# rogerhh/MonoGS

Hardware: AMD Instinct MI355X
Metric: rasteriser fwd+bwd fps @640x480/300k Gaussians (higher is better)
Workload: dtype f32; 1 GPU; SYN-C: 300000 Gaussians @ 640x480, SH degree 0, fwd+bwd incl. pose Jacobian through the autograd binding; pairs_D=750233, autograd_multithreading=False, parallelism=single view

## Files before the change

monogs_amd/csrc/raster_forward.hip:

```cpp
#include <type_traits>

#include "launch.h"
#include "raster_kernels.h"
#include "objective_math.h"
#define MGS_DIAG_FORWARD
#include "diag_stamp.h"

namespace mgs {

__device__ __forceinline__ void load_camera(Camera& c, const KP& P) {
#pragma unroll
  for (int i = 0; i < 16; i++) { c.V[i] = P.V[i]; c.PM[i] = P.PM[i]; c.Praw[i] = P.Praw[i]; }
  c.campos[0] = P.campos[0]; c.campos[1] = P.campos[1]; c.campos[2] = P.campos[2];
  c.W = P.W; c.H = P.H; c.tanfovx = P.tanfovx; c.tanfovy = P.tanfovy;
  c.focal_x = P.focal_x; c.focal_y = P.focal_y; c.scale_modifier = P.mod;
  c.sh_degree = P.deg; c.sh_coeffs = P.K; c.grid_x = P.grid_x; c.grid_y = P.grid_y;
  c.clamp_grad_upstream = P.clamp_up;
}

__device__ __forceinline__ void project_and_store(const KP& P, int idx, float4& r0, float4& r1) {
  Camera cam;
  load_camera(cam, P);
  const float p[3] = {P.means[3 * idx], P.means[3 * idx + 1], P.means[3 * idx + 2]};
  const float* pcol = P.precol ? P.precol + (size_t)3 * idx : nullptr;
// ... 186 lines not shown
          const int pos = P.tile_offset[t] + atomicAdd(&P.tile_cursor[t], 1);
          if (pos < P.cap) {
            P.keys[pos] = keyhi | (unsigned int)idx;
            P.payload[pos] = (unsigned int)cnt;
          }
        } else {
          atomicAdd(&P.tile_count[t], 1);
        }
        cnt++;
      }
    }
  }
  if (!emit) P.pair_count[idx] = cnt;
}

__global__ __launch_bounds__(256) void k_scan_reduce(KP P) {
  __shared__ int s[256];
  const int tid = threadIdx.x;
  const int base = blockIdx.x * kScanBlock + tid * 8;
  int sum = 0;
#pragma unroll
  for (int i = 0; i < 8; i++) sum += (base + i < P.N) ? P.pair_count[base + i] : 0;
  s[tid] = sum;
  __syncthreads();
  for (int off = 128; off > 0; off >>= 1) {
    if (tid < off) s[tid] += s[tid + off];
    __syncthreads();
  }
  if (tid == 0) P.scan_tmp[blockIdx.x] = s[0];
}

__global__ __launch_bounds__(1024) void k_scan_sums(KP P, int nblk) {
  __shared__ int s[1024];
  const int tid = threadIdx.x;
  int carry = 0;
  for (int base = 0; base < nblk; base += 1024) {
    const int i = base + tid;
    const int v = (i < nblk) ? P.scan_tmp[i] : 0;
    s[tid] = v;
    __syncthreads();
    for (int off = 1; off < 1024; off <<= 1) {
      const int t = (tid >= off) ? s[tid - off] : 0;
      __syncthreads();
      s[tid] += t;
      __syncthreads();
    }
    if (i < nblk) P.scan_tmp[i] = carry + s[tid] - v;
    carry += s[1023];
    __syncthreads();
  }
  if (tid == 0) P.scan_tmp[nblk] = carry;
}

__global__ __launch_bounds__(256) void k_scan_write(KP P) {
  __shared__ int s[256];
  const int tid = threadIdx.x;
  const int base = blockIdx.x * kScanBlock + tid * 8;
  int v[8], sum = 0;
#pragma unroll
  for (int i = 0; i < 8; i++) { v[i] = (base + i < P.N) ? P.pair_count[base + i] : 0; sum += v[i]; }
  s[tid] = sum;
  __syncthreads();
  for (int off = 1; off < 256; off <<= 1) {
    const int t = (tid >= off) ? s[tid - off] : 0;
    __syncthreads();
    s[tid] += t;
    __syncthreads();
  }
  int run = P.scan_tmp[blockIdx.x] + s[tid] - sum;
#pragma unroll
  for (int i = 0; i < 8; i++) {
    if (base + i < P.N) P.pair_off[base + i] = run;
    run += v[i];
  }
}

__device__ __forceinline__ void tile_scan_body(const KP& P, int nbin, int* s_sum, int* s_seg) {
  int* s_w = s_sum;
  const int tid = threadIdx.x, lane = tid & 63, wave = tid >> 6;
  const int vb = (nbin > 0 && tid < nbin) ? P.scan_tmp[tid] : 0;
  const int per = (P.T + 1023) / 1024;
  const int lo = tid * per, hi = min(lo + per, P.T);
  int local = 0, lseg = 0, lmax = 0;
  for (int i = lo; i < hi; i++) {
    const int c = __hip_atomic_load(&P.tile_count[i], __ATOMIC_RELAXED, __HIP_MEMORY_SCOPE_AGENT);
    local += c;
    lseg += (c + kItem - 1) / kItem;
    lmax = max(lmax, c);
  }
  int ib = vb, ip = local, is = lseg;
#pragma unroll
  for (int off = 1; off < 64; off <<= 1) {
    const int tb = __shfl_up(ib, off), tp = __shfl_up(ip, off), ts = __shfl_up(is, off);
    if (lane >= off) { ib += tb; ip += tp; is += ts; }
  }
#pragma unroll
  for (int off = 32; off > 0; off >>= 1) lmax = max(lmax, __shfl_xor(lmax, off));
  __syncthreads();
  if (lane == 63) { s_w[wave] = ib; s_w[16 + wave] = ip; s_w[32 + wave] = is; s_w[48 + wave] = lmax; }
  __syncthreads();
  int ob = 0, op = 0, os = 0, tot_p = 0, tot_s = 0, tmax = 0;
#pragma unroll
  for (int w = 0; w < 16; w++) {
    const int xb = s_w[w], xp = s_w[16 + w], xs = s_w[32 + w];
    if (w < wave) { ob += xb; op += xp; os += xs; }
    tot_p += xp; tot_s += xs;
    tmax = max(tmax, s_w[48 + w]);
  }
  if (nbin > 0) {
    if (tid < nbin) P.block_prefix[tid] = ob + ib - vb;
  } else if (tid == 0) {
    P.block_prefix[0] = 0;
  }
  int run = op + ip - local, rseg = os + is - lseg;
  for (int i = lo; i < hi; i++) {
    const int c = __hip_atomic_load(&P.tile_count[i], __ATOMIC_RELAXED, __HIP_MEMORY_SCOPE_AGENT);
    P.tile_offset[i] = run;
    P.seg_offset[i] = rseg;
    run += c;
    rseg += (c + kItem - 1) / kItem;
  }
  if (tid == 1023) {
    P.tile_offset[P.T] = tot_p;
    P.seg_offset[P.T] = tot_s;
    P.counters[0] = tot_p;
    if (P.d_out) {
      __hip_atomic_store(P.d_out + 1, tmax, __ATOMIC_RELAXED, __HIP_MEMORY_SCOPE_SYSTEM);
      __hip_atomic_store(P.d_out, tot_p, __ATOMIC_RELAXED, __HIP_MEMORY_SCOPE_SYSTEM);
    }
    P.counters[1] = tot_s;
    if (P.d_max) atomicMax(P.d_max, tot_p);
  }
  (void)s_seg;
}

__global__ __launch_bounds__(1024) void k_tile_scan(KP P, int nbin) {
  __shared__ int s_sum[1024], s_seg[1024];
  tile_scan_body(P, nbin, s_sum, s_seg);
}

constexpr int kColGroups = 16;
constexpr int kColRows = kBinBlocks / kColGroups;

__global__ __launch_bounds__(64 * kColGroups) void k_bin_colsum(KP P, int nblk) {
  __shared__ int s_sum2[2048];
  int (*s_sum)[64] = reinterpret_cast<int (*)[64]>(s_sum2);
  const int tl = threadIdx.x & 63, grp = threadIdx.x >> 6;
  const int t = blockIdx.x * 64 + tl;
  int v[kColRows];
  int sum = 0;
#pragma unroll
  for (int i = 0; i < kColRows; i++) {
    const int b = grp * kColRows + i;
    v[i] = (t < P.T && b < nblk) ? P.bin_table[(size_t)b * P.T + t] : 0;
    sum += v[i];
  }
  s_sum[grp][tl] = sum;
  __syncthreads();
  int run = 0, tot = 0;
#pragma unroll
  for (int g = 0; g < kColGroups; g++) {
    const int x = s_sum[g][tl];
    if (g < grp) run += x;
    tot += x;
  }
  if (t < P.T) {
#pragma unroll
    for (int i = 0; i < kColRows; i++) {
      const int b = grp * kColRows + i;
      if (b < nblk) P.bin_table[(size_t)b * P.T + t] = run;
      run += v[i];
    }
    if (grp == 0) __hip_atomic_store(&P.tile_count[t], tot, __ATOMIC_RELAXED, __HIP_MEMORY_SCOPE_AGENT);
  }
  __shared__ int s_last;
  if (threadIdx.x < 64) {
    asm volatile("s_waitcnt vmcnt(0)" ::: "memory");
    if (threadIdx.x == 0) {
      const int ticket = atomicAdd(&P.counters[3], 1);
      s_last = ticket == (int)gridDim.x - 1;
    }
  }
  __syncthreads();
  if (!s_last) return;
  tile_scan_body(P, nblk, s_sum2, s_sum2 + 1024);
}


template <bool WAVE_LOCAL, bool HAS_VAL, int NWAVES, typename KP_, typename VP_>
__device__ __forceinline__ void bitonic_sort(KP_ key, VP_ val, int n, int tid) {
  int m = 2;
  while (m < n) m <<= 1;
  const int half_m = m >> 1;
  const int nw = WAVE_LOCAL ? max(1, min(NWAVES, m >> 7)) : NWAVES;
  const int chunk = m / nw;
  const int cpw = half_m / nw;
  const int wave = tid >> 6, lane = tid & 63;
  const bool active = wave < nw;
  bool prev_global = true;
  auto sync = [&](bool global) {
    if (!WAVE_LOCAL || global || prev_global) {
      __syncthreads();
    } else {
      __builtin_amdgcn_fence(__ATOMIC_ACQ_REL, "wavefront");
      __builtin_amdgcn_wave_barrier();
    }
    prev_global = global;
  };
  constexpr int kMaxCmp = 2;
  auto run = [&](auto&& pair_of) {
    for (int c0 = 0; c0 < cpw; c0 += 64 * kMaxCmp) {
      int lo[kMaxCmp], hi[kMaxCmp];
      unsigned long long a[kMaxCmp], b[kMaxCmp];
      unsigned int va[kMaxCmp], vb[kMaxCmp];
#pragma unroll
      for (int u = 0; u < kMaxCmp; u++) {
        const int c = c0 + lane + 64 * u;
        lo[u] = -1;
        if (c < cpw) {
          pair_of(wave * cpw + c, lo[u], hi[u]);
          if (hi[u] >= n) lo[u] = -1;
        }
        if (lo[u] >= 0) {
          a[u] = key[lo[u]]; b[u] = key[hi[u]];
          if constexpr (HAS_VAL) { va[u] = val[lo[u]]; vb[u] = val[hi[u]]; }
        }
      }
#pragma unroll
      for (int u = 0; u < kMaxCmp; u++) {
        if (lo[u] >= 0 && a[u] > b[u]) {
          key[lo[u]] = b[u]; key[hi[u]] = a[u];
          if constexpr (HAS_VAL) { val[lo[u]] = vb[u]; val[hi[u]] = va[u]; }
        }
      }
    }
  };
  auto reg_pass = [&](bool first_rounds) {
    constexpr unsigned long long kInf = ~0ull;
    for (int e0 = 4 * lane; e0 < chunk; e0 += 256) {
      const int b0 = wave * chunk + e0;
      if (b0 >= n) continue;
      unsigned long long k4[4];
      unsigned int v4[4];
#pragma unroll
      for (int i = 0; i < 4; i++) {
        k4[i] = b0 + i < n ? key[b0 + i] : kInf;
        if constexpr (HAS_VAL) v4[i] = b0 + i < n ? val[b0 + i] : 0u;
      }
      auto ce = [&](int a, int b) {
        if (k4[a] > k4[b]) {
          const unsigned long long t = k4[a]; k4[a] = k4[b]; k4[b] = t;
          if constexpr (HAS_VAL) { const unsigned int u = v4[a]; v4[a] = v4[b]; v4[b] = u; }
        }
      };
      if (first_rounds) { ce(0, 1); ce(2, 3); ce(0, 3); ce(1, 2); ce(0, 1); ce(2, 3); }
      else { ce(0, 2); ce(1, 3); ce(0, 1); ce(2, 3); }
#pragma unroll
      for (int i = 0; i < 4; i++) {
        if (b0 + i < n) {
          key[b0 + i] = k4[i];
          if constexpr (HAS_VAL) val[b0 + i] = v4[i];
        }
      }
// ... 427 lines not shown
      for (int c = 0; c < 3; c++) {
        float dh;
        float r = om * (gain * im[c] + bias - gt[c]);
        if constexpr (DEPTH) r *= PD.w_rgb;
        l1 += fabsf(r);
        const float h = huber(r, P.obj.huber_delta, dh);
        float phi, gam;
        norm_terms(h, P.obj.p1 ? 1.f : 2.f, phi, gam);
        acc += phi;
        float gr = gam * dh * om;
        if constexpr (DEPTH) gr *= PD.w_rgb;
        ga += gr * im[c];
        gb += gr;
        P.obj.grad_image[c * HW + pix] = gr * gain;
      }
      if constexpr (DEPTH) {
        const float gtd = PD.gt_depth[pix];
        const float dm = (gtd > PD.depth_thr && 1.f - T > PD.opa_thr) ? 1.f : 0.f;
        const float rd = PD.w_depth * (C2D.y * dm - gtd * dm);
        float dh, phi, gam;
        l1 += fabsf(rd);
        const float h = huber(rd, P.obj.huber_delta, dh);
        norm_terms(h, P.obj.p1 ? 1.f : 2.f, phi, gam);
        acc += phi;
        PD.grad_depth[pix] = gam * dh * PD.w_depth * dm;
      }
    }
#pragma unroll
    for (int off = 32; off > 0; off >>= 1) {
      acc += __shfl_down(acc, off); ga += __shfl_down(ga, off); gb += __shfl_down(gb, off); l1 += __shfl_down(l1, off);
    }
    if (lane == 0) {
      const size_t n = 4 * (size_t)P.T;
      const float sgn = a > 0.f ? 1.f : (a < 0.f ? -1.f : 0.f);
      P.obj.partial[item] = acc;
      P.obj.partial[n + item] = ga * sgn;
      P.obj.partial[2 * n + item] = gb;
      P.obj.partial[3 * n + item] = l1;
    }
  }
}

template <bool OBJ>
__global__ __launch_bounds__(64, 6) void k_blend_fwd(KP P) { blend_fwd<OBJ, false>(P, KObjDepth{}); }

__global__ __launch_bounds__(64, 6) void k_blend_fwd_rgbd(KP P, KObjDepth PD) { blend_fwd<true, true>(P, PD); }

static inline int check_launch() {
  return launches_ok() ? MGS_OK : MGS_ERR_LAUNCH;
}

static inline int num_cus() {
  static int cus = 0;
  if (cus == 0) {
    int dev = 0, v = 0;
    cus = (hipGetDevice(&dev) == hipSuccess &&
           hipDeviceGetAttribute(&v, hipDeviceAttributeMultiprocessorCount, dev) == hipSuccess && v > 0) ? v : 256;
  }
  return cus;
}

static inline int bin_blocks(int N) {
  if (N <= kBinSmallMap) return max(1, (N + 255) / 256);
  int b = max(1, min(kBinBlocks, (N + 1023) / 1024));
  const int cus = num_cus();
  if (b > cus) b = b / cus * cus;
  return b;
}

void bin_grid(int N, int& nblk, int& per) {
  const int b = bin_blocks(N);
  per = ((N + b - 1) / b + kPreBlock - 1) / kPreBlock * kPreBlock;
  nblk = (N + per - 1) / per;
}

int launch_forward_project(const KP& P, hipStream_t st) {
  if (P.T <= kBinMaxTilesLds) {
    int nblk, per;
    bin_grid(P.N, nblk, per);
    if (P.N <= kBinSmallMap)
      launch_smem("project_bin_count", k_bin_lds<256>, dim3(nblk), dim3(256), sizeof(int) * (size_t)P.T, st, P, 0, per, 1);
    else
      launch_smem("project_bin_count", k_bin_lds<1024>, dim3(nblk), dim3(1024), sizeof(int) * (size_t)P.T, st, P, 0, per, 1);
    launch("bin_colsum", k_bin_colsum, dim3((P.T + 63) / 64), dim3(64 * kColGroups), st, P, nblk);
  } else {
    launch("preprocess", k_preprocess, dim3((P.N + kPreBlock - 1) / kPreBlock), dim3(kPreBlock), st, P);
    launch("bin_count", k_bin, dim3((P.N + 255) / 256), dim3(256), st, P, 0);
    const int nscan = (P.N + kScanBlock - 1) / kScanBlock;
    launch("scan_reduce", k_scan_reduce, dim3(nscan), dim3(256), st, P);
    launch("scan_sums", k_scan_sums, dim3(1), dim3(1024), st, P, nscan);
    launch("scan_write", k_scan_write, dim3(nscan), dim3(256), st, P);
    launch("tile_scan", k_tile_scan, dim3(1), dim3(1024), st, P, 0);
  }
  return check_launch();
}

int launch_forward_blend(const KP& P, hipStream_t st, const KObjDepth* PD) {
  if (P.T <= kBinMaxTilesLds) {
    int nblk, per;
    bin_grid(P.N, nblk, per);
    if (P.N <= kBinSmallMap)
      launch_smem("bin_emit", k_bin_lds<256>, dim3(nblk), dim3(256), sizeof(int) * (size_t)P.T, st, P, 1, per, 0);
    else
      launch_smem("bin_emit", k_bin_lds<1024>, dim3(nblk), dim3(1024), sizeof(int) * (size_t)P.T, st, P, 1, per, 0);
  } else {
    if (!hip_ok("memset(tile cursors)", hipMemsetAsync(P.tile_cursor, 0, sizeof(int) * (size_t)P.T, st)) ||
        !hip_ok("memset(n_touched)", hipMemsetAsync(P.n_touched, 0, sizeof(int) * (size_t)P.N, st))) {
      launches_ok();
      return MGS_ERR_LAUNCH;
    }
    launch("bin_emit", k_bin, dim3((P.N + 255) / 256), dim3(256), st, P, 1);
  }
  if (P.pack) {
    launch("tile_sort", k_tile_sort_reg<true>, dim3(P.T), dim3(256), st, P);
    if (P.big_pass) launch("tile_sort_big", k_tile_sort<4096, 1024, true, 1024>, dim3(min(P.T, 512)), dim3(1024), st, P);
  } else {
    launch("tile_sort", k_tile_sort_reg<false>, dim3(P.T), dim3(256), st, P);
    if (P.big_pass) launch("tile_sort_big", k_tile_sort<4096, 1024, false, 1024>, dim3(min(P.T, 512)), dim3(1024), st, P);
  }
#ifdef MGS_FWD_BLOCKS
  constexpr int kFwdGridChunk = 64;
#else
  constexpr int kFwdGridChunk = kFwdChunk;
#endif
  if (P.obj.on && PD && PD->gt_depth)
    launch("blend_fwd_rgbd", k_blend_fwd_rgbd, dim3(grid_pad(4 * P.T, kFwdGridChunk)), dim3(64), st, P, *PD);
  else if (P.obj.on) launch("blend_fwd", k_blend_fwd<true>, dim3(grid_pad(4 * P.T, kFwdGridChunk)), dim3(64), st, P);
  else launch("blend_fwd", k_blend_fwd<false>, dim3(grid_pad(4 * P.T, kFwdGridChunk)), dim3(64), st, P);
  return check_launch();
}

}
```

monogs_amd/csrc/tracking.hip:

```cpp
#include <hip/hip_runtime.h>

#include "../../include/monogs_raster.h"
#include "launch.h"
#include "objective_math.h"
#include "sketch_kernels.h"

namespace mgs {

__device__ inline void so3_exp_V(const float th[3], float R[9], float V[9]) {
  const float x = th[0], y = th[1], z = th[2];
  const float W[9] = {0.f, -z, y, z, 0.f, -x, -y, x, 0.f};
  float W2[9];
  for (int i = 0; i < 3; i++)
    for (int j = 0; j < 3; j++)
      W2[3 * i + j] = W[3 * i] * W[j] + W[3 * i + 1] * W[3 + j] + W[3 * i + 2] * W[6 + j];
  const float angle = sqrtf(x * x + y * y + z * z);
  float a, b, c, d;
  if (angle < 1e-5f) {
    a = 1.f; b = 0.5f; c = 0.5f; d = 1.f / 6.f;
  } else {
    const float s = sinf(angle), co = cosf(angle), a2 = angle * angle;
    a = s / angle; b = (1.f - co) / a2; c = b; d = (angle - s) / (a2 * angle);
  }
  for (int i = 0; i < 9; i++) {
// ... 124 lines not shown
#pragma unroll
    for (int i = 0; i < len[g]; i++) {
      const int o = first[g] + i;
      if (!on[o]) continue;
      m[o] = A.beta1 * m[o] + (1.f - A.beta1) * gr[o];
      v[o] = A.beta2 * v[o] + (1.f - A.beta2) * gr[o] * gr[o];
      const float denom = sqrtf(v[o]) / bc2s + A.eps;
      p[o] -= (lr[g] / bc1) * (m[o] / denom);
    }
  const bool move = have_T && !A.no_pose_update && A.cam_rot_delta && A.cam_trans_delta;
  const float th[3] = {move ? p[0] : 0.f, move ? p[1] : 0.f, move ? p[2] : 0.f};
  const float rho[3] = {move ? p[3] : 0.f, move ? p[4] : 0.f, move ? p[5] : 0.f};
  if (move) {
    float R[9], V[9];
    so3_exp_V(th, R, V);
    float t[3];
    for (int i = 0; i < 3; i++) t[i] = V[3 * i] * rho[0] + V[3 * i + 1] * rho[1] + V[3 * i + 2] * rho[2];
    float Tn[12];
    for (int i = 0; i < 3; i++)
      for (int j = 0; j < 4; j++)
        Tn[4 * i + j] = R[3 * i] * Tm[j] + R[3 * i + 1] * Tm[4 + j] + R[3 * i + 2] * Tm[8 + j] +
                        (j == 3 ? t[i] : 0.f) * Tm[15];
    for (int i = 0; i < 12; i++) Tm[i] = Tn[i];
    for (int i = 0; i < 6; i++) p[i] = 0.f;
  }
#pragma unroll
  for (int g = 0; g < 4; g++)
#pragma unroll
    for (int i = 0; i < len[g]; i++) {
      const int o = first[g] + i;
      if (on[o]) { A.exp_avg[o] = m[o]; A.exp_avg_sq[o] = v[o]; }
      if (on[o] || (move && o < 6)) P[g][i] = p[o];
    }
  if (A.best) {
    if (improved) {
      A.best[0] = s_l1;
#pragma unroll
      for (int i = 0; i < 18; i++) A.best[1 + i] = snap[i];
      A.best[19] = best_count;
    }
    A.best[20] = best_count + 1.f;
    if (A.l1_partials) A.best[21] = s_l1;
  }
  if (have_T) {
    if (move) for (int i = 0; i < 12; i++) A.T[i] = Tm[i];
    const float n2 = th[0] * th[0] + th[1] * th[1] + th[2] * th[2] + rho[0] * rho[0] + rho[1] * rho[1] +
                     rho[2] * rho[2];
    if (A.best) A.best[22] = sqrtf(n2);
    if (A.converged) *A.converged = n2 < A.converged_threshold * A.converged_threshold ? 1 : 0;
    if (want_mats) {
      for (int i = 0; i < 4; i++)
        for (int j = 0; j < 4; j++) {
          float acc = 0.f;
          for (int k = 0; k < 4; k++) acc += Tm[4 * k + i] * proj[4 * k + j];
          A.projmatrix_out[4 * i + j] = acc;
          A.viewmatrix_out[4 * i + j] = Tm[4 * j + i];
        }
    }
  }
}

__global__ void k_camera_from_pose(const float* T, const float* proj, float* view, float* full) {
  const int i = threadIdx.x >> 2, j = threadIdx.x & 3;
  if (threadIdx.x >= 16) return;
  float acc = 0.f;
  for (int k = 0; k < 4; k++) acc += T[4 * k + i] * proj[4 * k + j];
  const float v = T[4 * j + i];
  full[4 * i + j] = acc;
  view[4 * i + j] = v;
}

constexpr int kLossBlock = 256;
constexpr int kLossBlocks = 512;

__device__ __forceinline__ float block_sum(float v, float* s_red) {
  for (int off = 32; off > 0; off >>= 1) v += __shfl_down(v, off);
  const int lane = threadIdx.x & 63, wave = threadIdx.x >> 6;
  __syncthreads();
  if (lane == 0) s_red[wave] = v;
  __syncthreads();
  float t = 0.f;
  for (int w = 0; w < kLossBlock / 64; w++) t += s_red[w];
  return t;
}

__global__ __launch_bounds__(kLossBlock) void k_track_loss_fwd(mgs_tracking_loss_args A) {
  __shared__ float s_red[kLossBlock / 64];
  const float gain = fabsf(A.exposure_a[0]) + A.exposure_eps, bias = A.exposure_b[0];
  const float pn = norm_p(A.pnorm);
  const size_t HW = (size_t)A.num_pixels;
  float acc = 0.f;
  for (size_t p = (size_t)blockIdx.x * kLossBlock + threadIdx.x; p < HW; p += (size_t)gridDim.x * kLossBlock) {
    const float om = A.opacity[p] * (A.mask ? A.mask[p] : 1.f);
#pragma unroll
    for (int c = 0; c < 3; c++) {
      float dh, phi, gam;
      const float h = huber(om * (gain * A.image[c * HW + p] + bias - A.gt[c * HW + p]), A.huber_delta, dh);
      norm_terms(h, pn, phi, gam);
      acc += phi;
    }
  }
  const float t = block_sum(acc, s_red);
  if (threadIdx.x == 0) A.partial[blockIdx.x] = t;
}

__global__ __launch_bounds__(kLossBlock) void k_track_loss_finish(mgs_tracking_loss_args A, int nblk) {
  __shared__ float s_red[kLossBlock / 64];
  float acc = 0.f;
  for (int i = threadIdx.x; i < nblk; i += kLossBlock) acc += A.partial[i];
  const float t = block_sum(acc, s_red);
  if (threadIdx.x == 0) {
    float l, sc;
    norm_finish(t, norm_p(A.pnorm), l, sc);
    A.scalars[0] = l;
    A.scalars[1] = sc;
  }
}

__global__ __launch_bounds__(kLossBlock) void k_track_loss_bwd(mgs_tracking_loss_args A, int nfwd) {
  __shared__ float s_red[kLossBlock / 64];
  const float a = A.exposure_a[0];
  const float gain = fabsf(a) + A.exposure_eps, bias = A.exposure_b[0];
  const float sgn = a > 0.f ? 1.f : (a < 0.f ? -1.f : 0.f);
  const float pn = norm_p(A.pnorm);
  float inv_loss = 0.f;
  if (nfwd > 0) {
    float acc = 0.f;
    for (int i = threadIdx.x; i < nfwd; i += kLossBlock) acc += A.partial[i];
    float l;
    norm_finish(block_sum(acc, s_red), pn, l, inv_loss);
    if (blockIdx.x == 0 && threadIdx.x == 0) { A.scalars[0] = l; A.scalars[1] = inv_loss; }
    __syncthreads();
  } else {
    inv_loss = A.scalars[1];
  }
  const float k = A.grad_out[0] * inv_loss;
  const size_t HW = (size_t)A.num_pixels;
  float ga = 0.f, gb = 0.f;
  for (size_t p = (size_t)blockIdx.x * kLossBlock + threadIdx.x; p < HW; p += (size_t)gridDim.x * kLossBlock) {
    const float om = A.opacity[p] * (A.mask ? A.mask[p] : 1.f);
#pragma unroll
    for (int c = 0; c < 3; c++) {
      const float im = A.image[c * HW + p];
      float dh, phi, gam;
      const float h = huber(om * (gain * im + bias - A.gt[c * HW + p]), A.huber_delta, dh);
      norm_terms(h, pn, phi, gam);
      const float gr = k * gam * dh * om;
      A.grad_image[c * HW + p] = gr * gain;
      ga += gr * im;
      gb += gr;
    }
  }
  const float ta = block_sum(ga, s_red);
  const float tb = block_sum(gb, s_red);
  if (threadIdx.x == 0) {
    A.partial[nfwd + blockIdx.x] = ta * sgn;
    A.partial[nfwd + gridDim.x + blockIdx.x] = tb;
  }
}

__global__ __launch_bounds__(kLossBlock) void k_track_loss_bwd_finish(mgs_tracking_loss_args A, int nblk) {
  __shared__ float s_red[kLossBlock / 64];
  float x = 0.f, y = 0.f;
  for (int i = threadIdx.x; i < nblk; i += kLossBlock) { x += A.partial[i]; y += A.partial[nblk + i]; }
  const float ta = block_sum(x, s_red);
  const float tb = block_sum(y, s_red);
// ... 290 lines not shown
    if (s_last) __hip_atomic_store(ticket, 0, __ATOMIC_RELAXED, __HIP_MEMORY_SCOPE_AGENT);
  }
  __syncthreads();
  if (!s_last) return;
  const int nblk = gridDim.x;
  float x = 0.f, y = 0.f;
  for (int i = threadIdx.x; i < nblk; i += kLossBlock) {
    x += __hip_atomic_load(&A.partial[i], __ATOMIC_RELAXED, __HIP_MEMORY_SCOPE_AGENT);
    y += __hip_atomic_load(&A.partial[nblk + i], __ATOMIC_RELAXED, __HIP_MEMORY_SCOPE_AGENT);
  }
  const float sumc = block_sum(x, s_red);
  const float sumd = block_sum(y, s_red);
  if (threadIdx.x == 0) {
    const float hw = (float)A.num_pixels;
    A.loss[0] = A.w_rgb * sumc / (3.f * hw) + A.w_depth * sumd / hw;
  }
}

__global__ __launch_bounds__(kLossBlock) void k_map_loss_finish(mgs_mapping_loss_args A, int nblk) {
  __shared__ float s_red[kLossBlock / 64];
  float x = 0.f, y = 0.f;
  for (int i = threadIdx.x; i < nblk; i += kLossBlock) { x += A.partial[i]; y += A.partial[nblk + i]; }
  const float tc = block_sum(x, s_red);
  const float td = block_sum(y, s_red);
  if (threadIdx.x == 0) {
    const float hw = (float)A.num_pixels;
    A.loss[0] = A.w_rgb * tc / (3.f * hw) + A.w_depth * td / hw;
  }
}

__device__ __forceinline__ float sgn(float v) { return v > 0.f ? 1.f : (v < 0.f ? -1.f : 0.f); }

__global__ __launch_bounds__(kLossBlock) void k_map_loss_bwd(mgs_mapping_loss_args A) {
  __shared__ float s_red[kLossBlock / 64];
  const float a = A.apply_exposure ? A.exposure_a[0] : 1.f;
  const float gain = A.apply_exposure ? fabsf(a) + A.exposure_eps : 1.f;
  const float bias = A.apply_exposure ? A.exposure_b[0] : 0.f;
  const size_t HW = (size_t)A.num_pixels;
  const float hw = (float)A.num_pixels;
  const float kc = A.grad_out[0] * A.w_rgb / (3.f * hw), kd = A.grad_out[0] * A.w_depth / hw;
  float ga = 0.f, gb = 0.f;
  for (size_t p = (size_t)blockIdx.x * kLossBlock + threadIdx.x; p < HW; p += (size_t)gridDim.x * kLossBlock) {
    const float m = A.mask ? A.mask[p] : 1.f;
#pragma unroll
    for (int c = 0; c < 3; c++) {
      const float im = A.image[c * HW + p];
      const float g = kc * m * sgn(m * (gain * im + bias - A.gt[c * HW + p]));
      A.grad_image[c * HW + p] = g * gain;
      ga += g * im;
      gb += g;
    }
    if (A.grad_depth) {
      float g = 0.f;
      if (A.w_depth != 0.f) {
        const float gdp = A.gt_depth[p];
        const float dm = (A.depth_mask_threshold < 0.f || gdp > A.depth_mask_threshold) ? 1.f : 0.f;
        g = kd * dm * sgn(dm * (A.depth[p] - gdp));
      }
      A.grad_depth[p] = g;
    }
  }
  const float ta = block_sum(ga, s_red);
  const float tb = block_sum(gb, s_red);
  if (threadIdx.x == 0) {
    A.partial[blockIdx.x] = ta * sgn(a);
    A.partial[gridDim.x + blockIdx.x] = tb;
  }
}

__global__ __launch_bounds__(kLossBlock) void k_map_loss_bwd_finish(mgs_mapping_loss_args A, int nblk) {
  __shared__ float s_red[kLossBlock / 64];
  float x = 0.f, y = 0.f;
  for (int i = threadIdx.x; i < nblk; i += kLossBlock) { x += A.partial[i]; y += A.partial[nblk + i]; }
  const float ta = block_sum(x, s_red);
  const float tb = block_sum(y, s_red);
  if (threadIdx.x == 0) {
    if (A.grad_a) A.grad_a[0] = A.apply_exposure ? ta : 0.f;
    if (A.grad_b) A.grad_b[0] = A.apply_exposure ? tb : 0.f;
  }
}

template <bool VEC>
__global__ __launch_bounds__(kLossBlock) void k_map_loss_fused(mgs_mapping_loss_args A) {
  __shared__ float s_red[kLossBlock / 64];
  const float a = A.apply_exposure ? A.exposure_a[0] : 1.f;
  const float gain = A.apply_exposure ? fabsf(a) + A.exposure_eps : 1.f;
  const float bias = A.apply_exposure ? A.exposure_b[0] : 0.f;
  const size_t HW = (size_t)A.num_pixels;
  const float hw = (float)A.num_pixels;
  const float go = A.grad_out ? A.grad_out[0] : 1.f;
  const float kc = go * A.w_rgb / (3.f * hw), kd = go * A.w_depth / hw;
  float sc = 0.f, sd = 0.f, ga = 0.f, gb = 0.f;
  auto colour = [&](float m, float im, float gt) {
    const float r = m * (gain * im + bias - gt);
    sc += fabsf(r);
    const float g = kc * m * sgn(r);
    ga += g * im;
    gb += g;
    return g * gain;
  };
  auto depth = [&](float d, float gdp) {
    const float dm = (A.depth_mask_threshold < 0.f || gdp > A.depth_mask_threshold) ? 1.f : 0.f;
    const float r = dm * (d - gdp);
    sd += fabsf(r);
    return kd * dm * sgn(r);
  };
  if constexpr (VEC) {
    const size_t Q = HW / 4;
    const float4 one4 = make_float4(1.f, 1.f, 1.f, 1.f);
    for (size_t q = (size_t)blockIdx.x * kLossBlock + threadIdx.x; q < Q; q += (size_t)gridDim.x * kLossBlock) {
      const float4 m = A.mask ? reinterpret_cast<const float4*>(A.mask)[q] : one4;
      float4 im[3], gt[3];
#pragma unroll
      for (int c = 0; c < 3; c++) {
        im[c] = reinterpret_cast<const float4*>(A.image + c * HW)[q];
        gt[c] = reinterpret_cast<const float4*>(A.gt + c * HW)[q];
      }
      float4 dp = one4, gd = one4;
      const bool with_depth = A.w_depth != 0.f;
      if (with_depth) {
        dp = reinterpret_cast<const float4*>(A.depth)[q];
        gd = reinterpret_cast<const float4*>(A.gt_depth)[q];
      }
      float4 g[3], gdo = make_float4(0.f, 0.f, 0.f, 0.f);
#pragma unroll
      for (int c = 0; c < 3; c++) g[c].x = colour(m.x, im[c].x, gt[c].x);
      if (with_depth) gdo.x = depth(dp.x, gd.x);
#pragma unroll
      for (int c = 0; c < 3; c++) g[c].y = colour(m.y, im[c].y, gt[c].y);
      if (with_depth) gdo.y = depth(dp.y, gd.y);
#pragma unroll
      for (int c = 0; c < 3; c++) g[c].z = colour(m.z, im[c].z, gt[c].z);
      if (with_depth) gdo.z = depth(dp.z, gd.z);
#pragma unroll
      for (int c = 0; c < 3; c++) g[c].w = colour(m.w, im[c].w, gt[c].w);
      if (with_depth) gdo.w = depth(dp.w, gd.w);
#pragma unroll
      for (int c = 0; c < 3; c++) reinterpret_cast<float4*>(A.grad_image + c * HW)[q] = g[c];
      if (A.grad_depth) reinterpret_cast<float4*>(A.grad_depth)[q] = gdo;
    }
  } else {
    for (size_t p = (size_t)blockIdx.x * kLossBlock + threadIdx.x; p < HW; p += (size_t)gridDim.x * kLossBlock) {
      const float m = A.mask ? A.mask[p] : 1.f;
#pragma unroll
      for (int c = 0; c < 3; c++) A.grad_image[c * HW + p] = colour(m, A.image[c * HW + p], A.gt[c * HW + p]);
      if (A.w_depth != 0.f) {
        const float g = depth(A.depth[p], A.gt_depth[p]);
        if (A.grad_depth) A.grad_depth[p] = g;
      } else if (A.grad_depth) {
        A.grad_depth[p] = 0.f;
      }
    }
  }
  const float tc = block_sum(sc, s_red);
  const float td = block_sum(sd, s_red);
  const float ta = block_sum(ga, s_red);
  const float tb = block_sum(gb, s_red);
  const int n = gridDim.x;
  if (threadIdx.x == 0) {
    __hip_atomic_store(&A.partial[blockIdx.x], tc, __ATOMIC_RELAXED, __HIP_MEMORY_SCOPE_AGENT);
    __hip_atomic_store(&A.partial[n + blockIdx.x], td, __ATOMIC_RELAXED, __HIP_MEMORY_SCOPE_AGENT);
    __hip_atomic_store(&A.partial[2 * n + blockIdx.x], A.apply_exposure ? ta * sgn(a) : 0.f, __ATOMIC_RELAXED, __HIP_MEMORY_SCOPE_AGENT);
    __hip_atomic_store(&A.partial[3 * n + blockIdx.x], A.apply_exposure ? tb : 0.f, __ATOMIC_RELAXED, __HIP_MEMORY_SCOPE_AGENT);
  }
  if (!A.partial_ticket_ready) return;
  __shared__ int s_last;
  if (threadIdx.x == 0) {
    asm volatile("s_waitcnt vmcnt(0)" ::: "memory");
    int* ticket = reinterpret_cast<int*>(A.partial + 4 * n);
    s_last = atomicAdd(ticket, 1) == n - 1;
    if (s_last) __hip_atomic_store(ticket, 0, __ATOMIC_RELAXED, __HIP_MEMORY_SCOPE_AGENT);
  }
  __syncthreads();
  if (!s_last) return;
  float acc[4] = {0.f, 0.f, 0.f, 0.f};
  for (int i = threadIdx.x; i < n; i += kLossBlock)
#pragma unroll
    for (int c = 0; c < 4; c++) acc[c] += __hip_atomic_load(&A.partial[c * n + i], __ATOMIC_RELAXED, __HIP_MEMORY_SCOPE_AGENT);
  float tot[4];
#pragma unroll
  for (int c = 0; c < 4; c++) tot[c] = block_sum(acc[c], s_red);
  if (threadIdx.x == 0) {
    if (A.loss) A.loss[0] = A.w_rgb * tot[0] / (3.f * hw) + A.w_depth * tot[1] / hw;
    if (A.grad_a) A.grad_a[0] = tot[2];
    if (A.grad_b) A.grad_b[0] = tot[3];
  }
}


__global__ __launch_bounds__(256) void k_sketch_assign(long long m, int chunk, int d, int bits,
                                                       unsigned int k0, unsigned int k1, unsigned int k2,
                                                       int* bucket, float* weights) {
  const unsigned int mask = bits >= 32 ? 0xFFFFFFFFu : ((1u << bits) - 1u);
  for (long long p = (long long)blockIdx.x * 256 + threadIdx.x; p < m; p += (long long)gridDim.x * 256) {
    unsigned int x = (unsigned int)p;
    do { x = perm_round(x, mask, bits, k0, k1); } while ((long long)x >= m);
    const long long used = (long long)chunk * d;
    bucket[p] = (long long)x < used ? (int)(x / (unsigned int)chunk) : -1;
    weights[p] = (hash32((unsigned int)p ^ k2) & 0x10000u) ? 1.f : -1.f;
  }
}

__global__ __launch_bounds__(kSketchThreads) void k_sketch_residual(mgs_sketch_residual_args A, SketchKeys K) {
  extern __shared__ float s_acc[];
  __shared__ float s_red[kSketchThreads / 64];
  sketch_residual_block(A, K, s_acc, s_red, blockIdx.x, gridDim.x);
}

__global__ __launch_bounds__(kSketchThreads) void k_sketch_residual_rgbd(mgs_sketch_residual_args A, SketchKeys K,
                                                                        mgs_tracking_depth_args D) {
  extern __shared__ float s_acc[];
  __shared__ float s_red[kSketchThreads / 64];
  sketch_residual_block<true>(A, K, s_acc, s_red, blockIdx.x, gridDim.x, &D);
}

static int loss_blocks(int64_t hw) {
  const int64_t b = (hw + kLossBlock - 1) / kLossBlock;
  return (int)(b < kLossBlocks ? (b < 1 ? 1 : b) : kLossBlocks);
}

}

using namespace mgs;

extern "C" {

int32_t mgs_camera_from_pose(const float* T, const float* projection, float* viewmatrix,
                             float* projmatrix, void* stream) {
  if (!T || !projection || !viewmatrix || !projmatrix) return MGS_ERR_BAD_ARGUMENT;
  launch("camera_from_pose", k_camera_from_pose, dim3(1), dim3(64), (hipStream_t)stream, T, projection,
         viewmatrix, projmatrix);
  return launches_ok() ? MGS_OK : MGS_ERR_LAUNCH;
}

int32_t mgs_pose_adam_step(const mgs_pose_adam_args* a, void* stream) {
  if (!a || !a->exp_avg || !a->exp_avg_sq || a->step < 1) return MGS_ERR_BAD_ARGUMENT;
  if ((!a->cam_rot_delta || !a->cam_trans_delta) && !a->loss_partials && !a->exposure_partials && !a->grad_a && !a->grad_b)
    return MGS_ERR_BAD_ARGUMENT;
  if ((a->grad_a && !a->exposure_a) || (a->grad_b && !a->exposure_b)) return MGS_ERR_BAD_ARGUMENT;
  launch("pose_adam_update", k_pose_adam_update, dim3(1), dim3(512), (hipStream_t)stream, *a);
  return launches_ok() ? MGS_OK : MGS_ERR_LAUNCH;
}

static bool map_args_ok(const mgs_mapping_loss_args* a) {
  if (!a || !a->image || !a->gt || !a->partial || !a->loss || a->num_pixels < 1) return false;
  if (a->apply_exposure && (!a->exposure_a || !a->exposure_b)) return false;
  if (a->w_depth != 0.f && (!a->depth || !a->gt_depth)) return false;
  return true;
}

int32_t mgs_mapping_loss_forward(const mgs_mapping_loss_args* a, void* stream) {
  if (!map_args_ok(a)) return MGS_ERR_BAD_ARGUMENT;
  const int nb = loss_blocks(a->num_pixels);
  launch("map_loss_fwd", k_map_loss_fwd, dim3(nb), dim3(kLossBlock), (hipStream_t)stream, *a, a->partial_ticket_ready ? 1 : 0);
  if (!a->partial_ticket_ready)
    launch("map_loss_finish", k_map_loss_finish, dim3(1), dim3(kLossBlock), (hipStream_t)stream, *a, nb);
  return launches_ok() ? MGS_OK : MGS_ERR_LAUNCH;
}

int32_t mgs_mapping_loss_backward(const mgs_mapping_loss_args* a, void* stream) {
  if (!map_args_ok(a) || !a->grad_out || !a->grad_image) return MGS_ERR_BAD_ARGUMENT;
  const int nb = loss_blocks(a->num_pixels);
  launch("map_loss_bwd", k_map_loss_bwd, dim3(nb), dim3(kLossBlock), (hipStream_t)stream, *a);
  if (a->grad_a || a->grad_b)
// ... 147 lines not shown
```

Measured before the change: 3716 frames/s.

## Cut latency in tile scan, bin column-sum, and mapping loss reductions

```diff
diff --git a/monogs_amd/csrc/raster_forward.hip b/monogs_amd/csrc/raster_forward.hip
--- a/monogs_amd/csrc/raster_forward.hip
+++ b/monogs_amd/csrc/raster_forward.hip
@@ -292,11 +292,26 @@
   const int per = (P.T + 1023) / 1024;
   const int lo = tid * per, hi = min(lo + per, P.T);
   int local = 0, lseg = 0, lmax = 0;
-  for (int i = lo; i < hi; i++) {
-    const int c = __hip_atomic_load(&P.tile_count[i], __ATOMIC_RELAXED, __HIP_MEMORY_SCOPE_AGENT);
-    local += c;
-    lseg += (c + kItem - 1) / kItem;
-    lmax = max(lmax, c);
+  constexpr int kKeep = 4;
+  const bool keep = per <= kKeep;
+  int cnt[kKeep] = {0, 0, 0, 0};
+  if (keep) {
+#pragma unroll
+    for (int u = 0; u < kKeep; u++)
+      if (lo + u < hi) cnt[u] = __hip_atomic_load(&P.tile_count[lo + u], __ATOMIC_RELAXED, __HIP_MEMORY_SCOPE_AGENT);
+#pragma unroll
+    for (int u = 0; u < kKeep; u++) {
+      local += cnt[u];
+      lseg += (cnt[u] + kItem - 1) / kItem;
+      lmax = max(lmax, cnt[u]);
+    }
+  } else {
+    for (int i = lo; i < hi; i++) {
+      const int c = __hip_atomic_load(&P.tile_count[i], __ATOMIC_RELAXED, __HIP_MEMORY_SCOPE_AGENT);
+      local += c;
+      lseg += (c + kItem - 1) / kItem;
+      lmax = max(lmax, c);
+    }
   }
   int ib = vb, ip = local, is = lseg;
 #pragma unroll
@@ -323,12 +338,21 @@
     P.block_prefix[0] = 0;
   }
   int run = op + ip - local, rseg = os + is - lseg;
-  for (int i = lo; i < hi; i++) {
-    const int c = __hip_atomic_load(&P.tile_count[i], __ATOMIC_RELAXED, __HIP_MEMORY_SCOPE_AGENT);
-    P.tile_offset[i] = run;
-    P.seg_offset[i] = rseg;
-    run += c;
-    rseg += (c + kItem - 1) / kItem;
+  if (keep) {
+#pragma unroll
+    for (int u = 0; u < kKeep; u++) {
+      if (lo + u < hi) { P.tile_offset[lo + u] = run; P.seg_offset[lo + u] = rseg; }
+      run += cnt[u];
+      rseg += (cnt[u] + kItem - 1) / kItem;
+    }
+  } else {
+    for (int i = lo; i < hi; i++) {
+      const int c = __hip_atomic_load(&P.tile_count[i], __ATOMIC_RELAXED, __HIP_MEMORY_SCOPE_AGENT);
+      P.tile_offset[i] = run;
+      P.seg_offset[i] = rseg;
+      run += c;
+      rseg += (c + kItem - 1) / kItem;
+    }
   }
   if (tid == 1023) {
     P.tile_offset[P.T] = tot_p;
@@ -349,46 +373,59 @@
   tile_scan_body(P, nbin, s_sum, s_seg);
 }
 
-constexpr int kColGroups = 16;
+constexpr int kColTiles = 16;
+constexpr int kColGroups = 64;
 constexpr int kColRows = kBinBlocks / kColGroups;
-
-__global__ __launch_bounds__(64 * kColGroups) void k_bin_colsum(KP P, int nblk) {
+static_assert(kBinBlocks % kColGroups == 0 && kColTiles * kColGroups == 1024, "k_bin_colsum: 1024 threads");
+
+__global__ __launch_bounds__(kColTiles * kColGroups) void k_bin_colsum(KP P, int nblk) {
   __shared__ int s_sum2[2048];
-  int (*s_sum)[64] = reinterpret_cast<int (*)[64]>(s_sum2);
-  const int tl = threadIdx.x & 63, grp = threadIdx.x >> 6;
-  const int t = blockIdx.x * 64 + tl;
+  int (*s_wave)[kColTiles] = reinterpret_cast<int (*)[kColTiles]>(s_sum2);
+  const int lane = threadIdx.x & 63, wave = threadIdx.x >> 6;
+  const int tl = threadIdx.x & (kColTiles - 1), grp = threadIdx.x / kColTiles;
+  const int t = blockIdx.x * kColTiles + tl;
+  const int rows = (nblk + kColGroups - 1) / kColGroups;
+  const int b0 = grp * rows;
   int v[kColRows];
   int sum = 0;
 #pragma unroll
   for (int i = 0; i < kColRows; i++) {
-    const int b = grp * kColRows + i;
-    v[i] = (t < P.T && b < nblk) ? P.bin_table[(size_t)b * P.T + t] : 0;
+    const int b = b0 + i;
+    v[i] = (t < P.T && i < rows && b < nblk) ? P.bin_table[(size_t)b * P.T + t] : 0;
     sum += v[i];
   }
-  s_sum[grp][tl] = sum;
+  int inc = sum;
+  {
+    const int x = __shfl_up(inc, 16);
+    if (lane >= 16) inc += x;
+    const int y = __shfl_up(inc, 32);
+    if (lane >= 32) inc += y;
+  }
+  if (lane >= 48) s_wave[wave][tl] = inc;
   __syncthreads();
-  int run = 0, tot = 0;
-#pragma unroll
-  for (int g = 0; g < kColGroups; g++) {
-    const int x = s_sum[g][tl];
-    if (g < grp) run += x;
+  int run = inc - sum, tot = 0;
+#pragma unroll
+  for (int w = 0; w < 16; w++) {
+    const int x = s_wave[w][tl];
+    if (w < wave) run += x;
     tot += x;
-  }
-  if (t < P.T) {
-#pragma unroll
-    for (int i = 0; i < kColRows; i++) {
-      const int b = grp * kColRows + i;
-      if (b < nblk) P.bin_table[(size_t)b * P.T + t] = run;
-      run += v[i];
-    }
-    if (grp == 0) __hip_atomic_store(&P.tile_count[t], tot, __ATOMIC_RELAXED, __HIP_MEMORY_SCOPE_AGENT);
   }
   __shared__ int s_last;
   if (threadIdx.x < 64) {
+    if (threadIdx.x < kColTiles && t < P.T)
+      __hip_atomic_store(&P.tile_count[t], tot, __ATOMIC_RELAXED, __HIP_MEMORY_SCOPE_AGENT);
     asm volatile("s_waitcnt vmcnt(0)" ::: "memory");
     if (threadIdx.x == 0) {
       const int ticket = atomicAdd(&P.counters[3], 1);
       s_last = ticket == (int)gridDim.x - 1;
+    }
+  }
+  if (t < P.T) {
+#pragma unroll
+    for (int i = 0; i < kColRows; i++) {
+      const int b = b0 + i;
+      if (i < rows && b < nblk) P.bin_table[(size_t)b * P.T + t] = run;
+      run += v[i];
     }
   }
   __syncthreads();
@@ -982,7 +1019,7 @@
       launch_smem("project_bin_count", k_bin_lds<256>, dim3(nblk), dim3(256), sizeof(int) * (size_t)P.T, st, P, 0, per, 1);
     else
       launch_smem("project_bin_count", k_bin_lds<1024>, dim3(nblk), dim3(1024), sizeof(int) * (size_t)P.T, st, P, 0, per, 1);
-    launch("bin_colsum", k_bin_colsum, dim3((P.T + 63) / 64), dim3(64 * kColGroups), st, P, nblk);
+    launch("bin_colsum", k_bin_colsum, dim3((P.T + kColTiles - 1) / kColTiles), dim3(kColTiles * kColGroups), st, P, nblk);
   } else {
     launch("preprocess", k_preprocess, dim3((P.N + kPreBlock - 1) / kPreBlock), dim3(kPreBlock), st, P);
     launch("bin_count", k_bin, dim3((P.N + 255) / 256), dim3(256), st, P, 0);
diff --git a/monogs_amd/csrc/tracking.hip b/monogs_amd/csrc/tracking.hip
--- a/monogs_amd/csrc/tracking.hip
+++ b/monogs_amd/csrc/tracking.hip
@@ -230,6 +230,27 @@
   float t = 0.f;
   for (int w = 0; w < kLossBlock / 64; w++) t += s_red[w];
   return t;
+}
+
+__device__ __forceinline__ void block_sum4(float (&v)[4], float (*s_red4)[4]) {
+#pragma unroll
+  for (int off = 32; off > 0; off >>= 1) {
+#pragma unroll
+    for (int c = 0; c < 4; c++) v[c] += __shfl_down(v[c], off);
+  }
+  const int lane = threadIdx.x & 63, wave = threadIdx.x >> 6;
+  if (lane == 0) {
+#pragma unroll
+    for (int c = 0; c < 4; c++) s_red4[wave][c] = v[c];
+  }
+  __syncthreads();
+#pragma unroll
+  for (int c = 0; c < 4; c++) {
+    float t = 0.f;
+#pragma unroll
+    for (int w = 0; w < kLossBlock / 64; w++) t += s_red4[w][c];
+    v[c] = t;
+  }
 }
 
 __global__ __launch_bounds__(kLossBlock) void k_track_loss_fwd(mgs_tracking_loss_args A) {
@@ -686,7 +707,7 @@
 
 template <bool VEC>
 __global__ __launch_bounds__(kLossBlock) void k_map_loss_fused(mgs_mapping_loss_args A) {
-  __shared__ float s_red[kLossBlock / 64];
+  __shared__ float s_red4[2][kLossBlock / 64][4];
   const float a = A.apply_exposure ? A.exposure_a[0] : 1.f;
   const float gain = A.apply_exposure ? fabsf(a) + A.exposure_eps : 1.f;
   const float bias = A.apply_exposure ? A.exposure_b[0] : 0.f;
@@ -756,16 +777,14 @@
       }
     }
   }
-  const float tc = block_sum(sc, s_red);
-  const float td = block_sum(sd, s_red);
-  const float ta = block_sum(ga, s_red);
-  const float tb = block_sum(gb, s_red);
+  float t4[4] = {sc, sd, ga, gb};
+  block_sum4(t4, s_red4[0]);
   const int n = gridDim.x;
   if (threadIdx.x == 0) {
-    __hip_atomic_store(&A.partial[blockIdx.x], tc, __ATOMIC_RELAXED, __HIP_MEMORY_SCOPE_AGENT);
-    __hip_atomic_store(&A.partial[n + blockIdx.x], td, __ATOMIC_RELAXED, __HIP_MEMORY_SCOPE_AGENT);
-    __hip_atomic_store(&A.partial[2 * n + blockIdx.x], A.apply_exposure ? ta * sgn(a) : 0.f, __ATOMIC_RELAXED, __HIP_MEMORY_SCOPE_AGENT);
-    __hip_atomic_store(&A.partial[3 * n + blockIdx.x], A.apply_exposure ? tb : 0.f, __ATOMIC_RELAXED, __HIP_MEMORY_SCOPE_AGENT);
+    __hip_atomic_store(&A.partial[blockIdx.x], t4[0], __ATOMIC_RELAXED, __HIP_MEMORY_SCOPE_AGENT);
+    __hip_atomic_store(&A.partial[n + blockIdx.x], t4[1], __ATOMIC_RELAXED, __HIP_MEMORY_SCOPE_AGENT);
+    __hip_atomic_store(&A.partial[2 * n + blockIdx.x], A.apply_exposure ? t4[2] * sgn(a) : 0.f, __ATOMIC_RELAXED, __HIP_MEMORY_SCOPE_AGENT);
+    __hip_atomic_store(&A.partial[3 * n + blockIdx.x], A.apply_exposure ? t4[3] : 0.f, __ATOMIC_RELAXED, __HIP_MEMORY_SCOPE_AGENT);
   }
   if (!A.partial_ticket_ready) return;
   __shared__ int s_last;
@@ -777,13 +796,23 @@
   }
   __syncthreads();
   if (!s_last) return;
-  float acc[4] = {0.f, 0.f, 0.f, 0.f};
-  for (int i = threadIdx.x; i < n; i += kLossBlock)
-#pragma unroll
-    for (int c = 0; c < 4; c++) acc[c] += __hip_atomic_load(&A.partial[c * n + i], __ATOMIC_RELAXED, __HIP_MEMORY_SCOPE_AGENT);
-  float tot[4];
-#pragma unroll
-  for (int c = 0; c < 4; c++) tot[c] = block_sum(acc[c], s_red);
+  constexpr int kTrips = kLossBlocks / kLossBlock;
+  float ld[kTrips][4];
+#pragma unroll
+  for (int u = 0; u < kTrips; u++) {
+    const int i = min((int)threadIdx.x + u * kLossBlock, n - 1);
+#pragma unroll
+    for (int c = 0; c < 4; c++) ld[u][c] = __hip_atomic_load(&A.partial[c * n + i], __ATOMIC_RELAXED, __HIP_MEMORY_SCOPE_AGENT);
+  }
+  float tot[4] = {0.f, 0.f, 0.f, 0.f};
+#pragma unroll
+  for (int u = 0; u < kTrips; u++) {
+    if ((int)threadIdx.x + u * kLossBlock < n) {
+#pragma unroll
+      for (int c = 0; c < 4; c++) tot[c] += ld[u][c];
+    }
+  }
+  block_sum4(tot, s_red4[1]);
   if (threadIdx.x == 0) {
     if (A.loss) A.loss[0] = A.w_rgb * tot[0] / (3.f * hw) + A.w_depth * tot[1] / hw;
     if (A.grad_a) A.grad_a[0] = tot[2];
```

Measured after the change: 3735 frames/s (median of 5 runs). About the same (+0.5%).
